# HKUST-Aerial-Robotics/A-LOAM

Measured on AMD Instinct MI355X. Metric: HDL-64 scans/sec (whole node), higher is better.
Workload: dtype f32 features / f64 solve

## Files before the change

a-loam_amd/csrc/capi_internal.hpp:

```cpp
#pragma once
#include <hip/hip_runtime.h>

#include <cstdio>
#include <memory>
#include <string>
#include <utility>
#include <vector>

#include "../../include/aloam_mi355x.h"
#include "aloam_device.hpp"
#include "atlas_kernels.hpp"
#include "checkpoint_kernels.hpp"
#include "export_kernels.hpp"
#include "graphapply_kernels.hpp"
#include "graphmap_kernels.hpp"
#include "graphmarginal_kernels.hpp"
#include "loopreg_kernels.hpp"
#include "loopsearch_kernels.hpp"
#include "mapping_kernels.hpp"
#include "odometry_kernels.hpp"
#include "places_kernels.hpp"
#include "posegraph_kernels.hpp"
#include "registration_kernels.hpp"
#include "relocalize_kernels.hpp"

using namespace aloam;

// ... 350 lines not shown
  if (used[ns]) HIP_TRY(c, hipEventSynchronize(done[ns]));
  *slot = reinterpret_cast<T*>(mem.get() + (size_t)ns * slot_bytes);
  *index = ns;
  return ALOAM_OK;
}
template <int Slots>
int StageRing<Slots>::queue(aloam_ctx* c, int index, const void* src, size_t bytes, void* dst, hipStream_t stream) {
  HIP_TRY(c, hipMemcpyAsync(dst, src, bytes, hipMemcpyHostToDevice, stream));
  HIP_TRY(c, hipEventRecord(done[index], stream));
  used[index] = true;
  return ALOAM_OK;
}

inline float4* cloud_row(const aloam_ctx* c, const ExportSrc& s, int seq) {
  const int r = s.sel == kSelFixed ? 0 : s.sel == kSelCurrent ? c->seq[seq].parity : 1 - c->seq[seq].parity;
  return s.base[r] ? const_cast<float4*>(s.base[r]) + (size_t)seq * s.stride : nullptr;
}

int stage_ints(aloam_ctx* c, const int* src, int n, int* dst);
int check_seq(aloam_ctx* c, int seq);
int require_stage(aloam_ctx* c, int stage);
int check_ids(aloam_ctx* c, const int* ids, int n);
int register_launch(aloam_ctx* c, const void* d_scans, long long seq_stride, const int* n_in, int stride_bytes, int slot = -1, bool debug_arrays = true,
                    const int* n_cols = nullptr);
int stage_batch(aloam_ctx* c, const void* h_scans, long long seq_stride_bytes, size_t row, size_t last, size_t d_seq_stride, int* slot, char** d_in);
int ensure_dense(aloam_ctx* c);
long long cloud_desc(const aloam_ctx* c, int id, ExportSrc* s);
int find_cloud(aloam_ctx* c, int seq, int id, const float4** ptr, int* n);
OdomArgs odom_args(aloam_ctx* c);
MapArgs map_args(aloam_ctx* c);
int grow_map_pool(aloam_ctx* c, long long want, bool clamp);
void queue_map_spill(aloam_ctx* c, const int* mask);
int spill_dropped_since(aloam_ctx* c, long long* fresh);
int atlas_step_check(aloam_ctx* c);
bool queue_atlas_window(aloam_ctx* c, const int* mask);
long long largest_window(const std::vector<int>& keys, const std::vector<int>& counts, const int lo[3], const int hi[3], bool* exact);
KfStore kf_store(aloam_ctx* c);
int keyframe_add_check(aloam_ctx* c, const int* seqs, int n);
void queue_keyframe_capture(aloam_ctx* c, int n);
int queue_keyframe_rewind(aloam_ctx* c, const int* seqs, int n);
int keyframes_dropped_since(aloam_ctx* c, long long* fresh);
inline bool takes_part(const aloam_ctx* c, int b) { return c->all_active || c->seq[b].active; }
struct StageMask {
  std::vector<int> bits;
  const int* dev = nullptr;
  bool any_active = false, any_solve = false, all_solve = true, any_grow = false;
};
int stage_mask(aloam_ctx* c, DevBuf<int>& dst, int (*extra_bits)(const SeqHost&), bool (*unmasked)(const aloam_ctx*, const StageMask&), StageMask* m);
void on_active_mask_set(aloam_ctx* c, const int* active);
void on_frozen_mask_set(aloam_ctx* c, const int* frozen);
int on_slots_reset(aloam_ctx* c, const int* seqs, int n);
void on_slot_loaded(aloam_ctx* c, int seq, bool inited, long long err_events);
void on_sweep_registered(aloam_ctx* c);
void on_odometry_advanced(aloam_ctx* c, const StageMask& m);
void on_last_clouds_replaced(aloam_ctx* c, int seq);
void on_odometry_inputs_replaced(aloam_ctx* c, int seq);
void on_map_corrections_applied(aloam_ctx* c, const int* seqs, int n);
void on_system_inited_forced(aloam_ctx* c, int inited);
int on_map_replaced(aloam_ctx* c, int seq);
int on_map_pool_reallocated(aloam_ctx* c, MapPool&& fresh);
void on_mapping_step_queued(aloam_ctx* c);
int on_atlas_attached(aloam_ctx* c, const std::vector<int>& attached);
void on_places_enabled(aloam_ctx* c);
void on_descriptors_made(aloam_ctx* c, const int* seqs, int n);
void on_graph_nodes_added(aloam_ctx* c, const int* seqs, int n);
void on_graph_edges_added(aloam_ctx* c, int seq, int count);
void on_graph_cleared(aloam_ctx* c, const int* seqs, int n);
int on_graph_applied(aloam_ctx* c, const int* seqs, int n);
long long on_pool_events_reported(aloam_ctx* c, int seq, long long events);
int require_graph(aloam_ctx* c);
const char* graph_edge_check(const aloam_ctx* c, aloam_graph_edge& e, bool measurement);
VoxArgs vox_args(aloam_ctx* c, int n_segs, int levels);
enum CallerMem { kMemPageable, kMemDevice, kMemPinned, kMemManaged, kMemOtherDevice };
CallerMem classify_pointer(const aloam_ctx* c, const void* p, void** dev);
int require_host_list(aloam_ctx* c, const void* p, const char* name);
int export_target(aloam_ctx* c, const void* p, size_t align, const char* what, void** out);
int get_cube_list(aloam_ctx* c, int seq, int which, float* out, int cap_points);
// ... 3 lines not shown
```

a-loam_amd/csrc/capi_odometry.hip:

```cpp
#include <algorithm>
#include <cstring>

#include "capi_internal.hpp"

namespace {

RegArgs reg_args(aloam_ctx* c, const void* d_scans, long long seq_stride, int pt_stride) {
  RegArgs a{};
  a.in = (const char*)d_scans; a.seq_stride = seq_stride; a.pt_stride = pt_stride;
  a.B = c->B; a.cap = c->cap; a.R = c->R; a.NB = c->NB;
  a.ring_from_field = c->cfg.ring_from_field; a.min_range = c->cfg.min_range;
  a.meta = c->d_meta.get(); a.slabs = c->d_slabs.get(); a.slab = c->slab; a.front_lb = c->d_front_lb.get(); a.front_ticket = c->d_front_ticket.get();
  a.ringstart = c->d_ringstart.get(); a.cloud = c->d_cloud.get(); a.curv = c->d_curv.get(); a.label = c->d_label.get();
  a.lookback = c->d_lookback.get(); a.epoch = c->reg_epoch; a.store_debug = c->debug_arrays ? 1 : 0; a.ring_ticket = c->d_ring_ticket.get();
  a.sharp = c->d_sharp.get(); a.flat = c->d_flat.get();
  for (int k = 0; k < 2; ++k) { a.less_sharp[k] = c->d_less_sharp[k].get(); a.less_flat[k] = c->d_less_flat[k].get(); }
  a.active = c->reg_mask;
  return a;
}

}

namespace aloam {

// ... 16 lines not shown
  a.distortion = c->cfg.distortion != 0;
  return a;
}

}

namespace {

int check_batch(aloam_ctx* c, const int* n_in, int stride_bytes) {
  if (const int rc = require_stage(c, ALOAM_STAGE_REGISTRATION)) return rc;
  if (stride_bytes < 12 || (stride_bytes & 3)) { c->err = "stride_bytes must be 12 (x, y, z only) or >= 16, and a multiple of 4"; return ALOAM_E_ARG; }
  if (stride_bytes == 12 && c->cfg.ring_from_field) { c->err = "ring_from_field needs the 4th float of every record: stride_bytes >= 16"; return ALOAM_E_ARG; }
  for (int b = 0; b < c->B; ++b) {
    if (n_in[b] < 0) { c->err = "negative point count"; return ALOAM_E_ARG; }
    if (n_in[b] > c->max_points) { c->err = "scan exceeds max_points"; return ALOAM_E_CAPACITY; }
  }
  return ALOAM_OK;
}

}

namespace aloam {

int register_launch(aloam_ctx* c, const void* d_scans, long long seq_stride, const int* n_in, int stride_bytes, int slot, bool debug_arrays, const int* n_cols) {
  int rc = ALOAM_OK;
  if (!c->all_active && (rc = ensure_dense(c))) return rc;
  c->nin_max = 0;
  for (int b = 0; b < c->B; ++b) if (takes_part(c, b)) c->nin_max = std::max(c->nin_max, n_in[b]);
  if ((rc = stage_ints(c, n_cols ? n_cols : n_in, c->B, c->d_nin.get()))) return rc;
  if (n_cols) c->range_cols.assign(n_cols, n_cols + c->B); else c->range_cols.clear();
  StageMask m;
  rc = stage_mask(c, c->d_mask_reg, [](const SeqHost&) { return 0; }, [](const aloam_ctx* x, const StageMask&) { return x->all_active; }, &m);
  c->reg_mask = m.dev;
  if (rc) return rc;
  on_sweep_registered(c);
  c->debug_arrays = debug_arrays || c->sum_order != 0;
  if (((++c->reg_epoch) & 0x7fffffffu) == 0) ++c->reg_epoch;
  const RegArgs a = reg_args(c, d_scans, seq_stride, stride_bytes);
  if (n_cols) {
    const RangeArgs d{c->d_nin.get(), c->d_rd_az.get(), c->d_rd_rows.get(), c->rd_rows, c->rd_n_az, c->rd_order == ALOAM_RANGE_ROW_MAJOR ? 1 : 0, c->rd_scale};
    { ProfScope p(c, K_FIND_ENDS); launch_find_ends_range(a, d, c->stream); }
    { ProfScope p(c, K_FRONT); launch_front_range(a, d, c->stream); }
  } else {
    { ProfScope p(c, K_FIND_ENDS); launch_find_ends(a, c->d_nin.get(), c->stream); }
    { ProfScope p(c, K_FRONT); launch_front(a, c->stream); }
  }
  { ProfScope p(c, K_RING_STARTS); launch_ring_starts(a, c->stream); }
  c->dense_valid = false;
  if (slot >= 0) { HIP_TRY(c, hipEventRecord(c->in_consumed[slot], c->stream)); c->in_used[slot] = true; }
  { ProfScope p(c, K_RING_FEATURES); launch_ring_features(a, c->npad, 0.2f, c->stream);
    if (c->sum_order) launch_less_flat_reference_order(reg_args(c, d_scans, seq_stride, stride_bytes), c->npad, 0.2f, c->stream); }
  HIP_TRY(c, hipGetLastError());
  c->have_features = true;
  return ALOAM_OK;
}

int ensure_dense(aloam_ctx* c) {
  if (c->dense_valid) return ALOAM_OK;
  { ProfScope p(c, K_DENSE_CLOUD); launch_dense_cloud(reg_args(c, nullptr, 0, 16), c->stream); }
  HIP_TRY(c, hipGetLastError());
  c->dense_valid = true;
  return ALOAM_OK;
}

long long cloud_desc(const aloam_ctx* c, int id, ExportSrc* s) {
  const int* meta = reinterpret_cast<const int*>(c->d_meta.get());
  const int* mseq = reinterpret_cast<const int*>(c->d_mapseq.get());
  const int meta_ints = sizeof(SeqMeta) / sizeof(int), map_ints = sizeof(MapSeq) / sizeof(int);
  const long long sharp = (long long)c->R * kSharpPerRing, flat = (long long)c->R * kFlatPerRing, feat = (long long)c->R * kLessSharpPerRing;
// ... 38 lines not shown
  if (const int rc = c->d_in[s].grow(c, need)) return rc;
  *slot_out = s;
  return ALOAM_OK;
}

int stage_batch(aloam_ctx* c, const void* h_scans, long long seq_stride_bytes, size_t row, size_t last, size_t d_seq_stride, int* slot_out, char** d_in_out) {
  if (seq_stride_bytes < 0) { c->err = "bad stride"; return ALOAM_E_ARG; }
  if (c->B > 1 && (size_t)seq_stride_bytes < row) { c->err = "seq_stride_bytes smaller than a scan"; return ALOAM_E_ARG; }
  int slot = 0;
  if (const int rc = acquire_slab(c, d_seq_stride * c->B, &slot)) return rc;
  char* d_in = c->d_in[slot].get();
  if (row > 0) {
    if (c->B > 1) HIP_TRY(c, hipMemcpy2DAsync(d_in, d_seq_stride, h_scans, (size_t)seq_stride_bytes, row, (size_t)c->B - 1, hipMemcpyHostToDevice, c->copy_stream));
    if (last > 0) HIP_TRY(c, hipMemcpyAsync(d_in + (size_t)(c->B - 1) * d_seq_stride, (const char*)h_scans + (size_t)(c->B - 1) * (size_t)seq_stride_bytes, last, hipMemcpyHostToDevice, c->copy_stream));
  }
  HIP_TRY(c, hipEventRecord(c->in_copied[slot], c->copy_stream));
  HIP_TRY(c, hipStreamWaitEvent(c->stream, c->in_copied[slot], 0));
  *slot_out = slot; *d_in_out = d_in;
  return ALOAM_OK;
}

}

extern "C" {

int aloam_scan_register_device(aloam_ctx* c, const void* d_scans, long long seq_stride_bytes, const int* n_in, int stride_bytes) {
  DeviceScope device_scope(c);
  if (!c || !d_scans || !n_in) return ALOAM_E_ARG;
  if (const int rc = check_batch(c, n_in, stride_bytes)) return rc;
  return register_launch(c, d_scans, seq_stride_bytes, n_in, stride_bytes);
}

int aloam_scan_register(aloam_ctx* c, const void* const* scans, const int* n_in, int stride_bytes) {
  DeviceScope device_scope(c);
  if (!c || !scans || !n_in) return ALOAM_E_ARG;
  int rc = check_batch(c, n_in, stride_bytes);
  if (rc) return rc;
  const size_t seq_stride = (size_t)c->cap * stride_bytes;
  int slot = 0;
  if ((rc = acquire_slab(c, seq_stride * c->B, &slot))) return rc;
  char* d_in = c->d_in[slot].get();
  for (int b = 0; b < c->B; ++b)
    if (n_in[b] > 0) HIP_TRY(c, hipMemcpyAsync(d_in + b * seq_stride, scans[b], (size_t)n_in[b] * stride_bytes, hipMemcpyHostToDevice, c->stream));
  if ((rc = register_launch(c, d_in, (long long)seq_stride, n_in, stride_bytes, slot))) return rc;
  HIP_TRY(c, hipStreamSynchronize(c->stream));
  return ALOAM_OK;
}

static int stage_and_register(aloam_ctx* c, const void* h_scans, long long seq_stride_bytes, const int* n_in, int stride_bytes, bool debug_arrays) {
  if (!c || !h_scans || !n_in) return ALOAM_E_ARG;
  int rc = check_batch(c, n_in, stride_bytes);
  if (rc) return rc;
  const size_t d_seq_stride = (size_t)c->cap * stride_bytes;
  int slot = 0;
  char* d_in = nullptr;
  if ((rc = stage_batch(c, h_scans, seq_stride_bytes, (size_t)*std::max_element(n_in, n_in + c->B) * stride_bytes, (size_t)n_in[c->B - 1] * stride_bytes, d_seq_stride, &slot, &d_in))) return rc;
  return register_launch(c, d_in, (long long)d_seq_stride, n_in, stride_bytes, slot, debug_arrays);
}

int aloam_scan_register_host(aloam_ctx* c, const void* h_scans, long long seq_stride_bytes, const int* n_in, int stride_bytes) {
  DeviceScope device_scope(c);
  return stage_and_register(c, h_scans, seq_stride_bytes, n_in, stride_bytes, true);
}

int aloam_process_host(aloam_ctx* c, const void* h_scans, long long seq_stride_bytes, const int* n_in, int stride_bytes) {
  DeviceScope device_scope(c);
  const int rc = stage_and_register(c, h_scans, seq_stride_bytes, n_in, stride_bytes, false);
  if (rc) return rc;
  return aloam_odometry_step(c);
}

int aloam_input_consumed(aloam_ctx* c) {
  DeviceScope device_scope(c);
  if (!c) return ALOAM_E_ARG;
  for (int s = 0; s < 2; ++s) if (c->in_used[s]) HIP_TRY(c, hipEventSynchronize(c->in_consumed[s]));
  return ALOAM_OK;
}

int aloam_odometry_step(aloam_ctx* c) {
  DeviceScope device_scope(c);
  if (!c) return ALOAM_E_ARG;
  if (const int rc = require_stage(c, ALOAM_STAGE_ODOMETRY)) return rc;
  if (!c->have_features) { c->err = "aloam_odometry_step before any features were registered / set"; return ALOAM_E_STATE; }
  StageMask m;
  if (const int rc = stage_mask(c, c->d_mask_odo, [](const SeqHost& s) { return s.inited ? (int)kSeqSolve : 0; },
                                [](const aloam_ctx* x, const StageMask& k) { return k.all_solve || (!k.any_solve && x->all_active); }, &m)) return rc;
  const int* mask = m.dev;
  const bool any_solve = m.any_solve;
  const bool overlap = c->grid_overlap;
  bool build_last = !overlap;
  if (overlap) for (int b = 0; b < c->B; ++b) build_last |= (m.bits[b] & kSeqSolve) && !c->seq[b].grid_built;
  hipError_t join_err = hipSuccess;
  const int cus = c->gather_blocks / 8;
  auto launch_all = [&]() {
    OdomArgs a = odom_args(c);
    a.active = mask;
    if (overlap) {
      hipError_t e = hipEventRecord(c->grid_fork, c->stream);
      if (e == hipSuccess) e = hipStreamWaitEvent(c->grid_stream, c->grid_fork, 0);
      { ProfScope p(c, K_BUILD_GRIDS, c->grid_stream); launch_build_grids(a, true, cus, c->grid_stream); }
      if (e == hipSuccess) e = hipEventRecord(c->grids_done, c->grid_stream);
      join_err = e;
    }
    if (any_solve && build_last) {
      if (overlap) launch_build_grids(a, false, cus, c->stream);
      else { ProfScope p(c, K_BUILD_GRIDS); launch_build_grids(a, false, cus, c->stream); }
    }
    for (int outer = 0; any_solve && outer < c->cfg.outer_iterations; ++outer) {
      a.outer = outer;
      a.last_outer = outer == c->cfg.outer_iterations - 1;
      { ProfScope p(c, K_TRANSFORM); launch_transform_queries(a, c->stream); }
      { ProfScope p(c, K_ASSOC_CORNER); launch_associate(a, false, c->stream); }
      { ProfScope p(c, K_ASSOC_PLANE); launch_associate(a, true, c->stream); }
      { ProfScope p(c, K_SOLVE); launch_solve(a, c->stream); }
    }
    if (overlap && join_err == hipSuccess) join_err = hipStreamWaitEvent(c->stream, c->grids_done, 0);
    { ProfScope p(c, K_ADVANCE); launch_advance(a, c->stream); }
  };
  if (!any_solve) {
    launch_all();
  } else if (c->use_graph && !c->prof_on && !c->debug_sync) {
    GraphExec& ge = c->odom_graph[mask ? 1 : 0];
    if (!ge) {
      hipGraph_t g = nullptr;
      hipError_t e = hipStreamBeginCapture(c->stream, hipStreamCaptureModeThreadLocal);
      if (e == hipSuccess) {
        launch_all();
        e = hipStreamEndCapture(c->stream, &g);
        if (e == hipSuccess) e = hipGraphInstantiate(&ge.h, g, nullptr, nullptr, 0);
        if (g) (void)hipGraphDestroy(g);
      }
      if (e != hipSuccess) {
        (void)hipGetLastError();
        ge.reset();
        c->use_graph = false;
      }
    }
    if (ge) HIP_TRY(c, hipGraphLaunch(ge, c->stream));
    else launch_all();
  } else {
    launch_all();
  }
  HIP_TRY(c, join_err);
  HIP_TRY(c, hipGetLastError());
  on_odometry_advanced(c, m);
  return ALOAM_OK;
}

int aloam_process_device(aloam_ctx* c, const void* d_scans, long long seq_stride_bytes, const int* n_in, int stride_bytes) {
  DeviceScope device_scope(c);
  if (!c || !d_scans || !n_in) return ALOAM_E_ARG;
  int rc = check_batch(c, n_in, stride_bytes);
  if (rc || (rc = register_launch(c, d_scans, seq_stride_bytes, n_in, stride_bytes, -1, false))) return rc;
  return aloam_odometry_step(c);
}

int aloam_cloud_size(aloam_ctx* c, int seq, int which) {
  DeviceScope device_scope(c);
  const float4* p; int n;
  const int rc = find_cloud(c, seq, which < ALOAM_EXPORT_MAP ? which : -1, &p, &n);
  return rc ? rc : n;
}

int aloam_get_cloud(aloam_ctx* c, int seq, int which, float* out, int cap_points) {
  DeviceScope device_scope(c);
  const float4* p; int n;
  if (const int rc = find_cloud(c, seq, which < ALOAM_EXPORT_MAP ? which : -1, &p, &n)) return rc;
  const int k = n < cap_points ? n : cap_points;
  if (k > 0) HIP_TRY(c, hipMemcpy(out, p, sizeof(float4) * k, hipMemcpyDeviceToHost));
  return n;
}

int aloam_get_pose(aloam_ctx* c, int seq, double q_w[4], double t_w[3], double q_lc[4], double t_lc[3]) {
  DeviceScope device_scope(c);
  int rc = check_seq(c, seq);
  if (rc) return rc;
  OdomState s;
// ... 176 lines not shown
```

a-loam_amd/csrc/capi_seq.hip:

```cpp
#include "capi_internal.hpp"

static int mark_window_stale(aloam_ctx* c, int seq) {
  if (c->any_attached && c->seq[seq].attached) HIP_TRY(c, hipMemsetAsync(c->d_at_stale.get() + seq, 1, sizeof(int), c->stream));
  return ALOAM_OK;
}

namespace aloam {

int stage_mask(aloam_ctx* c, DevBuf<int>& dst, int (*extra_bits)(const SeqHost&), bool (*unmasked)(const aloam_ctx*, const StageMask&), StageMask* m) {
  m->bits.resize(c->B);
  for (int b = 0; b < c->B; ++b) {
    const int v = m->bits[b] = takes_part(c, b) ? (kSeqActive | extra_bits(c->seq[b])) : 0;
    m->any_active |= v != 0; m->any_grow |= (v & kSeqMapGrow) != 0;
    m->any_solve |= (v & kSeqSolve) != 0; m->all_solve &= (v & kSeqSolve) != 0;
  }
  if (unmasked(c, *m)) return ALOAM_OK;
  if (!dst && dmalloc(c, dst, c->B)) return ALOAM_E_HIP;
  if (const int rc = stage_ints(c, m->bits.data(), c->B, dst.get())) return rc;
  m->dev = dst.get();
  return ALOAM_OK;
}

void on_active_mask_set(aloam_ctx* c, const int* active) {
  c->all_active = true;
// ... 22 lines not shown
    SeqHost& s = c->seq[seqs[i]];
    s.parity = 0; s.inited = 0; s.grid_built = false; s.needs_odom = false; s.map_err_seen = 0; s.scorable = false; s.has_sweep = false; s.desc_valid = false;
    s.info_odom = false; s.info_map = false; s.has_stacks = false;
  }
  for (int i = 0; i < n; ++i) if (const int rc = mark_window_stale(c, seqs[i])) return rc;
  return ALOAM_OK;
}

void on_slot_loaded(aloam_ctx* c, int seq, bool inited, long long err_events) {
  SeqHost& s = c->seq[seq];
  s.inited = inited; s.map_err_seen = err_events; s.needs_odom = (c->stages & ALOAM_STAGE_ODOMETRY) != 0;
}

void on_sweep_registered(aloam_ctx* c) {
  const bool odo = c->stages & ALOAM_STAGE_ODOMETRY;
  for (int b = 0; b < c->B; ++b) {
    SeqHost& s = c->seq[b];
    if (odo) s.reg_active = s.active;
    if (takes_part(c, b)) { s.has_sweep = true; s.desc_valid = false; s.info_odom = false; }
  }
  if (odo) c->reg_pending = true;
}

void on_odometry_advanced(aloam_ctx* c, const StageMask& m) {
  for (int b = 0; b < c->B; ++b) {
    SeqHost& s = c->seq[b];
    if (m.bits[b] & kSeqActive) {
      s.parity ^= 1; s.inited = 1; s.needs_odom = false; s.grid_built = c->grid_overlap;
      s.info_odom = (m.bits[b] & kSeqSolve) && c->cfg.outer_iterations > 0;
    }
  }
  c->reg_pending = false;
}

void on_last_clouds_replaced(aloam_ctx* c, int seq) { c->seq[seq].grid_built = false; c->seq[seq].info_odom = false; }
void on_odometry_inputs_replaced(aloam_ctx* c, int seq) { c->seq[seq].info_odom = false; }

int on_map_replaced(aloam_ctx* c, int seq) {
  HIP_TRY(c, hipMemsetAsync(c->d_grid_sig.get() + (size_t)seq * 2, 0, sizeof(MapGridSig) * 2, c->stream));
  c->seq[seq].scorable = false; c->seq[seq].info_map = false;
  return mark_window_stale(c, seq);
}

int on_map_pool_reallocated(aloam_ctx* c, MapPool&& fresh) {
  if (c->d_grid_sig) HIP_TRY(c, hipMemsetAsync(c->d_grid_sig.get(), 0, sizeof(MapGridSig) * c->B * 2, c->stream));
  HIP_TRY(c, hipStreamSynchronize(c->stream));
  c->map = std::move(fresh);
  for (SeqHost& s : c->seq) s.scorable = false;
  return ALOAM_OK;
}

// ... 37 lines not shown
```

a-loam_amd/csrc/odometry_kernels.hip:

```cpp
#include "aloam_device.hpp"
#include "aloam_trig.hpp"
#include "lm_device.hpp"
#include "odometry_solve_device.hpp"
#include "odometry_kernels.hpp"

namespace aloam {

#define ALOAM_PHASE(name) asm volatile("; ##PHASE " name)
#ifdef ALOAM_PHASE_CLOCK
__device__ unsigned long long g_phase_clock_odo[2][32];
#define ALOAM_BG_CLOCK(slot) do { if (threadIdx.x == 0 && blockIdx.x == 1) { atomicAdd(&g_phase_clock_odo[0][slot], (unsigned long long)__builtin_readcyclecounter()); atomicAdd(&g_phase_clock_odo[1][slot], 1ull); } } while (0)
#else
#define ALOAM_BG_CLOCK(slot) do { } while (0)
#endif
#ifdef ALOAM_ASSOC_STATS
__device__ unsigned long long g_assoc_stats[2][32];
#define ALOAM_STAT(cls, i, v) do { if ((threadIdx.x & 63) == 0) atomicAdd(&g_assoc_stats[cls][i], (unsigned long long)(v)); } while (0)
#else
#define ALOAM_STAT(cls, i, v) do { } while (0)
#endif

__device__ __forceinline__ float4 transform_to_start(const float4& p, const OdomState& st) {
  double q[4] = {st.para_q[0], st.para_q[1], st.para_q[2], st.para_q[3]};
  if (q[3] < 0.0) { q[0] = -q[0]; q[1] = -q[1]; q[2] = -q[2]; q[3] = -q[3]; }
// ... 165 lines not shown
#pragma unroll
      for (int t = 0; t < 3; ++t) {
        const unsigned sh = (h[t] & 1u) * 16;
        pos[t] = (atomicAdd(&tab[t * (H / 2) + (h[t] >> 1)], 1u << sh) >> sh) & 0xffffu;
      }
      const float4 e = make_float4(p[u].x, p[u].y, p[u].z, __uint_as_float((unsigned)i | ((unsigned)(key + 1) << 20)));
      g.sorted3[pos[0]] = e;
      g.sorted3c[pos[1]] = e;
      g.sorted2[pos[2]] = e;
    }
  }
  ALOAM_BG_CLOCK(5);
#ifdef ALOAM_PHASE_CLOCK
  __syncthreads();
  ALOAM_BG_CLOCK(6);
#endif
}

__global__ __launch_bounds__(1024) void k_build_grids_fused(OdomArgs a) { build_grids_fused<false>(a, blockIdx.y, blockIdx.x); }
__global__ __launch_bounds__(1024) void k_build_grids_fused_next(OdomArgs a) {
  const int G = gridDim.x;
  for (int r = 0, i = blockIdx.x; i < 2 * a.B; ++r, i += G) {
    build_grids_fused<true>(a, i >> 1, (i ^ r) & 1);
    __syncthreads();
  }
}

constexpr int kBgWaves = 4;
constexpr int kBgUnroll = 4;
template <bool NEXT>
__device__ __forceinline__ void build_grids(const OdomArgs& a) {
  constexpr int U = kBgUnroll;
  const int b = blockIdx.y, which = blockIdx.x / 3, tid = threadIdx.x;
  const int pass_lo = blockIdx.x % 3, pass_hi = pass_lo + 1;
  if (seq_idle(a.active, b, NEXT ? kSeqActive : kSeqSolve)) return;
  const SeqMeta m = a.meta[b];
  const BuildSrc<NEXT> src(a, m, b, which);
  const int n = src.n;
  const float4* pts = src.pts;
  const GridView g = grid_view(a, b, which, src.set);
  if (fused_takes(n, g.H)) return;
  extern __shared__ __attribute__((aligned(16))) int lds[];
  int* cnt = lds;
  int* part = lds + g.H;
  int* s_flag = part + 1024;
  if (tid < 2) s_flag[tid] = n >= (1 << 20) && tid == 0 ? 1 : 0;
// ... 901 lines not shown
  }
}

__global__ void k_advance(SeqMeta* meta, OdomState* state, const int* active, int B) {
  const int b = blockIdx.x * blockDim.x + threadIdx.x;
  if (b >= B || seq_idle(active, b)) return;
  SeqMeta& m = meta[b];
  m.n_corner_last = m.n_less_sharp; m.n_surf_last = m.n_less_flat; m.parity ^= 1;
  state[b].inited = 1;
}
__global__ void k_set_inited(OdomState* state, int B, int inited) {
  const int b = blockIdx.x * blockDim.x + threadIdx.x;
  if (b < B) state[b].inited = inited;
}
void launch_set_inited(OdomState* state, int B, int inited, hipStream_t s) { hipLaunchKernelGGL(k_set_inited, dim3((B + 63) / 64), dim3(64), 0, s, state, B, inited); }
void launch_advance(const OdomArgs& a, hipStream_t s) { hipLaunchKernelGGL(k_advance, dim3((a.B + 63) / 64), dim3(64), 0, s, a.meta, a.state, a.active, a.B); }

size_t build_grids_lds_bytes(int H, int R) { return sizeof(int) * ((size_t)H + 1024 + 2 * (R + 8) + 4); }
static size_t build_grids_fused_lds_bytes(int H) { return sizeof(int) * (3 * (size_t)(H / 2) + 48 + 8 + 2 * kWalkKeys); }
int prepare_build_grids(int H_surf) {
  const int fused = (int)build_grids_fused_lds_bytes(kFusedMaxH), per_grid = (int)build_grids_lds_bytes(H_surf, kMaxRings);
  if (hipFuncSetAttribute((const void*)k_build_grids_fused, hipFuncAttributeMaxDynamicSharedMemorySize, fused) != hipSuccess) return -1;
  if (hipFuncSetAttribute((const void*)k_build_grids_fused_next, hipFuncAttributeMaxDynamicSharedMemorySize, fused) != hipSuccess) return -1;
  if (hipFuncSetAttribute((const void*)k_build_grids, hipFuncAttributeMaxDynamicSharedMemorySize, per_grid) != hipSuccess) return -1;
  return hipFuncSetAttribute((const void*)k_build_grids_next, hipFuncAttributeMaxDynamicSharedMemorySize, per_grid) == hipSuccess ? 0 : -1;
}
void launch_build_grids(const OdomArgs& a, bool next, int cus, hipStream_t s) {
  const int hc = a.grid_H_corner <= kFusedMaxH ? a.grid_H_corner : 0, hs = a.grid_H_surf <= kFusedMaxH ? a.grid_H_surf : 0;
  const size_t fused = build_grids_fused_lds_bytes(hc > hs ? hc : hs), per_grid = build_grids_lds_bytes(a.grid_H_surf, a.R);
  if (next) {
    const int wgs = cus / 2 >= 2 ? (cus / 2) & ~1 : 2;
    if (hc || hs) hipLaunchKernelGGL(k_build_grids_fused_next, dim3(2 * a.B < wgs ? 2 * a.B : wgs), dim3(1024), fused, s, a);
    hipLaunchKernelGGL(k_build_grids_next, dim3(6, a.B), dim3(1024), per_grid, s, a);
  } else {
    if (hc || hs) hipLaunchKernelGGL(k_build_grids_fused, dim3(2, a.B), dim3(1024), fused, s, a);
    hipLaunchKernelGGL(k_build_grids, dim3(6, a.B), dim3(1024), per_grid, s, a);
  }
}
void launch_transform_queries(const OdomArgs& a, hipStream_t s) {
  const dim3 grid((a.R * (kSharpPerRing + kFlatPerRing) + 255) / 256, a.B);
  if (a.distortion) hipLaunchKernelGGL(k_transform_queries<true>, grid, dim3(256), 0, s, a);
  else hipLaunchKernelGGL(k_transform_queries<false>, grid, dim3(256), 0, s, a);
}
void launch_associate(const OdomArgs& a, bool plane, hipStream_t s) {
  const int by = (a.B + 7) / 8 * 8;
  const int qcap = plane ? a.R * kFlatPerRing : a.R * kSharpPerRing;
  const bool wide = a.R > 64;
  const dim3 grid((unsigned)(qcap / 2 * by)), block(64), gridf((unsigned)a.B), blockf(256);
  const dim3 gridn((unsigned)((qcap / 2 + kPairsPerWave - 1) / kPairsPerWave), (unsigned)a.B);
  if (wide) {
    if (plane) { hipLaunchKernelGGL((k_associate_pair<true, true>), grid, block, 0, s, a); hipLaunchKernelGGL((k_associate_nearly<true, true>), gridn, block, 0, s, a); hipLaunchKernelGGL((k_associate_flagged<true, true>), gridf, blockf, 0, s, a); }
    else { hipLaunchKernelGGL((k_associate_pair<false, true>), grid, block, 0, s, a); hipLaunchKernelGGL((k_associate_nearly<false, true>), gridn, block, 0, s, a); hipLaunchKernelGGL((k_associate_flagged<false, true>), gridf, blockf, 0, s, a); }
  } else {
    if (plane) { hipLaunchKernelGGL((k_associate_pair<true, false>), grid, block, 0, s, a); hipLaunchKernelGGL((k_associate_nearly<true, false>), gridn, block, 0, s, a); hipLaunchKernelGGL((k_associate_flagged<true, false>), gridf, blockf, 0, s, a); }
    else { hipLaunchKernelGGL((k_associate_pair<false, false>), grid, block, 0, s, a); hipLaunchKernelGGL((k_associate_nearly<false, false>), gridn, block, 0, s, a); hipLaunchKernelGGL((k_associate_flagged<false, false>), gridf, blockf, 0, s, a); }
  }
}
void launch_solve(const OdomArgs& a, hipStream_t s) {
  if (a.distortion) hipLaunchKernelGGL(k_solve<true>, dim3(a.B), dim3(kSolveThreads), 0, s, a);
// ... 11 lines not shown
```

a-loam_amd/csrc/odometry_kernels.hpp:

```cpp
#pragma once
#include "aloam_device.hpp"

struct aloam_pose_information;

namespace aloam {
size_t build_grids_lds_bytes(int H, int R);
int prepare_build_grids(int H_surf);
void launch_build_grids(const OdomArgs& a, bool next, int cus, hipStream_t s);
void launch_transform_queries(const OdomArgs& a, hipStream_t s);
void launch_associate(const OdomArgs& a, bool plane, hipStream_t s);
void launch_solve(const OdomArgs& a, hipStream_t s);
void launch_advance(const OdomArgs& a, hipStream_t s);
void launch_pose_information_odom(const OdomArgs& a, const int* list, int n, aloam_pose_information* dst, hipStream_t s);
void launch_set_inited(OdomState* state, int B, int inited, hipStream_t s);
}
```

a-loam_amd/csrc/registration_kernels.hip:

```cpp
#include "aloam_device.hpp"
#include "registration_kernels.hpp"
#include "voxel_device.hpp"

namespace aloam {

struct RecordLoader {
  static constexpr bool kKeepPoint = true;
  const char* in; int stride;
  __device__ __forceinline__ float4 operator()(int i) const { return load_point(in, i, stride); }
};

#ifndef ALOAM_RANGE_KEEP_POINT
#define ALOAM_RANGE_KEEP_POINT 0
#endif
struct RangeLoader {
  static constexpr bool kKeepPoint = ALOAM_RANGE_KEEP_POINT;
  const unsigned short* az; const unsigned short* range;
  const float2* az_xy; const float* tab;
  unsigned div, magic; int n_az; bool row_major; float scale;
  __device__ __forceinline__ float4 operator()(int i) const {
#ifdef ALOAM_RANGE_PHASES
    asm volatile("; ##PHASE decode");
#endif
    const unsigned code = range[i];
// ... 30 lines not shown
  __shared__ int s_first, s_last;
  if (tid == 0) { s_first = 0x7fffffff; s_last = -1; }
  __syncthreads();
  for (int base = 0; base < n; base += 4096) {
    bool any = false;
#pragma unroll
    for (int k = 0; k < 4; ++k) {
      const int i = base + k * 1024 + tid;
      if (i < n && point_kept(load(i), a.min_range)) { atomicMin(&s_first, i); any = true; }
    }
    if (__syncthreads_or(any)) break;
  }
  for (int base = 0; base < n; base += 4096) {
    bool any = false;
#pragma unroll
    for (int k = 0; k < 4; ++k) {
      const int i = n - 1 - (base + k * 1024 + tid);
      if (i >= 0 && point_kept(load(i), a.min_range)) { atomicMax(&s_last, i); any = true; }
    }
    if (__syncthreads_or(any)) break;
  }
  __syncthreads();
  if (tid == 0) {
    SeqMeta m = a.meta[b];
    m.n_in = n;
    m.first_kept = s_first;
    m.last_kept = s_last;
    m.half_idx = 0x7fffffff;
    m.err = 0;
    m.n_cloud = 0;
    m.start_ori = 0.f;
    m.end_ori = 0.f;
    if (s_last < 0) {
      m.err = kErrEmpty;
    } else {
      const float4 p0 = load(s_first);
      const float4 p1 = load(s_last);
      const float startOri = -atan2f_port(p0.y, p0.x);
      float endOri = (float)((double)(-atan2f_port(p1.y, p1.x)) + 2 * M_PI);
      if ((double)(endOri - startOri) > 3 * M_PI) endOri = (float)((double)endOri - 2 * M_PI);
      else if ((double)(endOri - startOri) < M_PI) endOri = (float)((double)endOri + 2 * M_PI);
      m.start_ori = startOri;
      m.end_ori = endOri;
    }
    if (n > a.cap) m.err |= kErrPointCap;
    a.meta[b] = m;
  }
}
__global__ __launch_bounds__(1024) void k_find_ends(RegArgs a, const int* __restrict__ n_in) {
  const int b = blockIdx.x;
  if (seq_idle(a.active, b)) return;
  find_ends_body(a, b, n_in[b], RecordLoader{a.in + (long long)b * a.seq_stride, a.pt_stride});
}

__device__ __forceinline__ int ring_from_angle(float angle, int R) {
  int scanID;
  if (R == 16) {
    scanID = (int)((double)((angle + 15) / 2) + 0.5);
    return (scanID > R - 1 || scanID < 0) ? -1 : scanID;
  }
  if (R == 32) {
    scanID = (int)(((double)angle + 92.0 / 3.0) * 3.0 / 4.0);
    return (scanID > R - 1 || scanID < 0) ? -1 : scanID;
  }
  if ((double)angle >= -8.83) scanID = (int)((double)(2 - angle) * 3.0 + 0.5);
  else scanID = R / 2 + (int)((-8.83 - (double)angle) * 2.0 + 0.5);
  if ((double)angle > 2 || (double)angle < -24.33 || scanID > 50 || scanID < 0) return -1;
  return scanID;
}
// ... 769 lines not shown
```

Measured before the change: 133,300.

## Overlap last-cloud grid build with scan registration on a side stream

In the fused process paths, when sequences need their previous-cloud grids built, the build is forked onto the grid stream right after the registration front kernel. It runs with a fixed workgroup budget, so it overlaps the rest of registration instead of running serially at the start of odometry. The odometry step then skips its own next-grid overlap and joins the fork before advancing. This adds a new persistent 'last' kernel variant and a std::function callback, and risks contention between the two streams. It also makes find_ends write only the SeqMeta fields it changes, through a reference, instead of copying the whole struct.

```diff
diff --git a/a-loam_amd/csrc/capi_internal.hpp b/a-loam_amd/csrc/capi_internal.hpp
--- a/a-loam_amd/csrc/capi_internal.hpp
+++ b/a-loam_amd/csrc/capi_internal.hpp
@@ -3,6 +3,7 @@
 
 #include <cstdio>
 #include <memory>
+#include <functional>
 #include <string>
 #include <utility>
 #include <vector>
@@ -399,7 +400,7 @@
 int require_stage(aloam_ctx* c, int stage);
 int check_ids(aloam_ctx* c, const int* ids, int n);
 int register_launch(aloam_ctx* c, const void* d_scans, long long seq_stride, const int* n_in, int stride_bytes, int slot = -1, bool debug_arrays = true,
-                    const int* n_cols = nullptr);
+                    const int* n_cols = nullptr, const std::function<void()>* after_front = nullptr);
 int stage_batch(aloam_ctx* c, const void* h_scans, long long seq_stride_bytes, size_t row, size_t last, size_t d_seq_stride, int* slot, char** d_in);
 int ensure_dense(aloam_ctx* c);
 long long cloud_desc(const aloam_ctx* c, int id, ExportSrc* s);
@@ -429,7 +430,7 @@
 int on_slots_reset(aloam_ctx* c, const int* seqs, int n);
 void on_slot_loaded(aloam_ctx* c, int seq, bool inited, long long err_events);
 void on_sweep_registered(aloam_ctx* c);
-void on_odometry_advanced(aloam_ctx* c, const StageMask& m);
+void on_odometry_advanced(aloam_ctx* c, const StageMask& m, bool built_next);
 void on_last_clouds_replaced(aloam_ctx* c, int seq);
 void on_odometry_inputs_replaced(aloam_ctx* c, int seq);
 void on_map_corrections_applied(aloam_ctx* c, const int* seqs, int n);
diff --git a/a-loam_amd/csrc/capi_odometry.hip b/a-loam_amd/csrc/capi_odometry.hip
--- a/a-loam_amd/csrc/capi_odometry.hip
+++ b/a-loam_amd/csrc/capi_odometry.hip
@@ -1,5 +1,6 @@
 #include <algorithm>
 #include <cstring>
+#include <functional>
 
 #include "capi_internal.hpp"
 
@@ -62,7 +63,8 @@
 
 namespace aloam {
 
-int register_launch(aloam_ctx* c, const void* d_scans, long long seq_stride, const int* n_in, int stride_bytes, int slot, bool debug_arrays, const int* n_cols) {
+int register_launch(aloam_ctx* c, const void* d_scans, long long seq_stride, const int* n_in, int stride_bytes, int slot, bool debug_arrays, const int* n_cols,
+                    const std::function<void()>* after_front) {
   int rc = ALOAM_OK;
   if (!c->all_active && (rc = ensure_dense(c))) return rc;
   c->nin_max = 0;
@@ -85,6 +87,7 @@
     { ProfScope p(c, K_FIND_ENDS); launch_find_ends(a, c->d_nin.get(), c->stream); }
     { ProfScope p(c, K_FRONT); launch_front(a, c->stream); }
   }
+  if (after_front) (*after_front)();
   { ProfScope p(c, K_RING_STARTS); launch_ring_starts(a, c->stream); }
   c->dense_valid = false;
   if (slot >= 0) { HIP_TRY(c, hipEventRecord(c->in_consumed[slot], c->stream)); c->in_used[slot] = true; }
@@ -169,89 +172,92 @@
 
 }
 
-extern "C" {
-
-int aloam_scan_register_device(aloam_ctx* c, const void* d_scans, long long seq_stride_bytes, const int* n_in, int stride_bytes) {
-  DeviceScope device_scope(c);
-  if (!c || !d_scans || !n_in) return ALOAM_E_ARG;
-  if (const int rc = check_batch(c, n_in, stride_bytes)) return rc;
-  return register_launch(c, d_scans, seq_stride_bytes, n_in, stride_bytes);
-}
-
-int aloam_scan_register(aloam_ctx* c, const void* const* scans, const int* n_in, int stride_bytes) {
-  DeviceScope device_scope(c);
-  if (!c || !scans || !n_in) return ALOAM_E_ARG;
-  int rc = check_batch(c, n_in, stride_bytes);
-  if (rc) return rc;
-  const size_t seq_stride = (size_t)c->cap * stride_bytes;
-  int slot = 0;
-  if ((rc = acquire_slab(c, seq_stride * c->B, &slot))) return rc;
-  char* d_in = c->d_in[slot].get();
-  for (int b = 0; b < c->B; ++b)
-    if (n_in[b] > 0) HIP_TRY(c, hipMemcpyAsync(d_in + b * seq_stride, scans[b], (size_t)n_in[b] * stride_bytes, hipMemcpyHostToDevice, c->stream));
-  if ((rc = register_launch(c, d_in, (long long)seq_stride, n_in, stride_bytes, slot))) return rc;
-  HIP_TRY(c, hipStreamSynchronize(c->stream));
-  return ALOAM_OK;
-}
-
-static int stage_and_register(aloam_ctx* c, const void* h_scans, long long seq_stride_bytes, const int* n_in, int stride_bytes, bool debug_arrays) {
-  if (!c || !h_scans || !n_in) return ALOAM_E_ARG;
-  int rc = check_batch(c, n_in, stride_bytes);
-  if (rc) return rc;
-  const size_t d_seq_stride = (size_t)c->cap * stride_bytes;
-  int slot = 0;
-  char* d_in = nullptr;
-  if ((rc = stage_batch(c, h_scans, seq_stride_bytes, (size_t)*std::max_element(n_in, n_in + c->B) * stride_bytes, (size_t)n_in[c->B - 1] * stride_bytes, d_seq_stride, &slot, &d_in))) return rc;
-  return register_launch(c, d_in, (long long)d_seq_stride, n_in, stride_bytes, slot, debug_arrays);
-}
-
-int aloam_scan_register_host(aloam_ctx* c, const void* h_scans, long long seq_stride_bytes, const int* n_in, int stride_bytes) {
-  DeviceScope device_scope(c);
-  return stage_and_register(c, h_scans, seq_stride_bytes, n_in, stride_bytes, true);
-}
-
-int aloam_process_host(aloam_ctx* c, const void* h_scans, long long seq_stride_bytes, const int* n_in, int stride_bytes) {
-  DeviceScope device_scope(c);
-  const int rc = stage_and_register(c, h_scans, seq_stride_bytes, n_in, stride_bytes, false);
-  if (rc) return rc;
-  return aloam_odometry_step(c);
-}
-
-int aloam_input_consumed(aloam_ctx* c) {
-  DeviceScope device_scope(c);
-  if (!c) return ALOAM_E_ARG;
-  for (int s = 0; s < 2; ++s) if (c->in_used[s]) HIP_TRY(c, hipEventSynchronize(c->in_consumed[s]));
-  return ALOAM_OK;
-}
-
-int aloam_odometry_step(aloam_ctx* c) {
-  DeviceScope device_scope(c);
-  if (!c) return ALOAM_E_ARG;
+namespace {
+
+struct GridFork {
+  aloam_ctx* c;
+  bool open = false;
+  hipError_t err = hipSuccess;
+  explicit GridFork(aloam_ctx* c_) : c(c_) {}
+  GridFork(const GridFork&) = delete;
+  GridFork& operator=(const GridFork&) = delete;
+  ~GridFork() { join(); }
+  void note(hipError_t e) { if (err == hipSuccess) err = e; }
+  void begin() {
+    const hipError_t e = hipEventRecord(c->grid_fork, c->stream);
+    note(e);
+    if (e == hipSuccess) note(hipStreamWaitEvent(c->grid_stream, c->grid_fork, 0));
+    open = true;
+  }
+  void launched() { note(hipEventRecord(c->grids_done, c->grid_stream)); }
+  void join() {
+    if (open && err == hipSuccess) note(hipStreamWaitEvent(c->stream, c->grids_done, 0));
+    open = false;
+  }
+};
+
+constexpr int kGridWgsBesideRegistration = 96;
+
+struct OdomStep {
+  StageMask m;
+  bool masked = false;
+  bool beside_registration = false;
+  bool build = false;
+  GridFork fork;
+  explicit OdomStep(aloam_ctx* c) : fork(c) {}
+};
+
+int odometry_mask(aloam_ctx* c, OdomStep* st) {
+  if (const int rc = stage_mask(c, c->d_mask_odo, [](const SeqHost& s) { return s.inited ? (int)kSeqSolve : 0; },
+                                [](const aloam_ctx* x, const StageMask& k) { return k.all_solve || (!k.any_solve && x->all_active); }, &st->m)) return rc;
+  st->masked = true;
+  return ALOAM_OK;
+}
+
+int odometry_begin(aloam_ctx* c, OdomStep* st) {
+  if (!(c->stages & ALOAM_STAGE_ODOMETRY) || !c->grid_overlap) return ALOAM_OK;
+  if (const int rc = odometry_mask(c, st)) return rc;
+  st->beside_registration = true;
+  for (int b = 0; b < c->B; ++b) st->build |= (st->m.bits[b] & kSeqSolve) && !c->seq[b].grid_built;
+  return ALOAM_OK;
+}
+
+void odometry_fork_build(aloam_ctx* c, OdomStep* st) {
+  OdomArgs a = odom_args(c);
+  a.active = st->m.dev;
+  st->fork.begin();
+  { ProfScope p(c, K_BUILD_GRIDS, c->grid_stream); launch_build_grids(a, GridBuild::kPersistentLast, kGridWgsBesideRegistration, c->grid_stream); }
+  st->fork.launched();
+}
+
+int register_with_step(aloam_ctx* c, OdomStep* st, const void* d_scans, long long seq_stride, const int* n_in, int stride_bytes, int slot) {
+  const std::function<void()> fork = [c, st]() { odometry_fork_build(c, st); };
+  return register_launch(c, d_scans, seq_stride, n_in, stride_bytes, slot, false, nullptr, st->build ? &fork : nullptr);
+}
+
+int odometry_finish(aloam_ctx* c, OdomStep* st) {
   if (const int rc = require_stage(c, ALOAM_STAGE_ODOMETRY)) return rc;
   if (!c->have_features) { c->err = "aloam_odometry_step before any features were registered / set"; return ALOAM_E_STATE; }
-  StageMask m;
-  if (const int rc = stage_mask(c, c->d_mask_odo, [](const SeqHost& s) { return s.inited ? (int)kSeqSolve : 0; },
-                                [](const aloam_ctx* x, const StageMask& k) { return k.all_solve || (!k.any_solve && x->all_active); }, &m)) return rc;
+  if (!st->masked) if (const int rc = odometry_mask(c, st)) return rc;
+  const StageMask& m = st->m;
   const int* mask = m.dev;
   const bool any_solve = m.any_solve;
-  const bool overlap = c->grid_overlap;
-  bool build_last = !overlap;
+  st->fork.join();
+  const bool overlap = c->grid_overlap && !st->beside_registration;
+  bool build_last = !c->grid_overlap;
   if (overlap) for (int b = 0; b < c->B; ++b) build_last |= (m.bits[b] & kSeqSolve) && !c->seq[b].grid_built;
-  hipError_t join_err = hipSuccess;
   const int cus = c->gather_blocks / 8;
   auto launch_all = [&]() {
     OdomArgs a = odom_args(c);
     a.active = mask;
     if (overlap) {
-      hipError_t e = hipEventRecord(c->grid_fork, c->stream);
-      if (e == hipSuccess) e = hipStreamWaitEvent(c->grid_stream, c->grid_fork, 0);
-      { ProfScope p(c, K_BUILD_GRIDS, c->grid_stream); launch_build_grids(a, true, cus, c->grid_stream); }
-      if (e == hipSuccess) e = hipEventRecord(c->grids_done, c->grid_stream);
-      join_err = e;
+      st->fork.begin();
+      { ProfScope p(c, K_BUILD_GRIDS, c->grid_stream); launch_build_grids(a, GridBuild::kPersistentNext, cus / 2, c->grid_stream); }
+      st->fork.launched();
     }
     if (any_solve && build_last) {
-      if (overlap) launch_build_grids(a, false, cus, c->stream);
-      else { ProfScope p(c, K_BUILD_GRIDS); launch_build_grids(a, false, cus, c->stream); }
+      if (overlap) launch_build_grids(a, GridBuild::kSerialLast, 0, c->stream);
+      else { ProfScope p(c, K_BUILD_GRIDS); launch_build_grids(a, GridBuild::kSerialLast, 0, c->stream); }
     }
     for (int outer = 0; any_solve && outer < c->cfg.outer_iterations; ++outer) {
       a.outer = outer;
@@ -261,7 +267,7 @@
       { ProfScope p(c, K_ASSOC_PLANE); launch_associate(a, true, c->stream); }
       { ProfScope p(c, K_SOLVE); launch_solve(a, c->stream); }
     }
-    if (overlap && join_err == hipSuccess) join_err = hipStreamWaitEvent(c->stream, c->grids_done, 0);
+    st->fork.join();
     { ProfScope p(c, K_ADVANCE); launch_advance(a, c->stream); }
   };
   if (!any_solve) {
@@ -288,18 +294,86 @@
   } else {
     launch_all();
   }
-  HIP_TRY(c, join_err);
+  HIP_TRY(c, st->fork.err);
   HIP_TRY(c, hipGetLastError());
-  on_odometry_advanced(c, m);
-  return ALOAM_OK;
+  on_odometry_advanced(c, m, overlap);
+  return ALOAM_OK;
+}
+
+}
+
+extern "C" {
+
+int aloam_scan_register_device(aloam_ctx* c, const void* d_scans, long long seq_stride_bytes, const int* n_in, int stride_bytes) {
+  DeviceScope device_scope(c);
+  if (!c || !d_scans || !n_in) return ALOAM_E_ARG;
+  if (const int rc = check_batch(c, n_in, stride_bytes)) return rc;
+  return register_launch(c, d_scans, seq_stride_bytes, n_in, stride_bytes);
+}
+
+int aloam_scan_register(aloam_ctx* c, const void* const* scans, const int* n_in, int stride_bytes) {
+  DeviceScope device_scope(c);
+  if (!c || !scans || !n_in) return ALOAM_E_ARG;
+  int rc = check_batch(c, n_in, stride_bytes);
+  if (rc) return rc;
+  const size_t seq_stride = (size_t)c->cap * stride_bytes;
+  int slot = 0;
+  if ((rc = acquire_slab(c, seq_stride * c->B, &slot))) return rc;
+  char* d_in = c->d_in[slot].get();
+  for (int b = 0; b < c->B; ++b)
+    if (n_in[b] > 0) HIP_TRY(c, hipMemcpyAsync(d_in + b * seq_stride, scans[b], (size_t)n_in[b] * stride_bytes, hipMemcpyHostToDevice, c->stream));
+  if ((rc = register_launch(c, d_in, (long long)seq_stride, n_in, stride_bytes, slot))) return rc;
+  HIP_TRY(c, hipStreamSynchronize(c->stream));
+  return ALOAM_OK;
+}
+
+static int stage_and_register(aloam_ctx* c, const void* h_scans, long long seq_stride_bytes, const int* n_in, int stride_bytes, bool debug_arrays, OdomStep* step = nullptr) {
+  if (!c || !h_scans || !n_in) return ALOAM_E_ARG;
+  int rc = check_batch(c, n_in, stride_bytes);
+  if (rc || (step && (rc = odometry_begin(c, step)))) return rc;
+  const size_t d_seq_stride = (size_t)c->cap * stride_bytes;
+  int slot = 0;
+  char* d_in = nullptr;
+  if ((rc = stage_batch(c, h_scans, seq_stride_bytes, (size_t)*std::max_element(n_in, n_in + c->B) * stride_bytes, (size_t)n_in[c->B - 1] * stride_bytes, d_seq_stride, &slot, &d_in))) return rc;
+  if (step) return register_with_step(c, step, d_in, (long long)d_seq_stride, n_in, stride_bytes, slot);
+  return register_launch(c, d_in, (long long)d_seq_stride, n_in, stride_bytes, slot, debug_arrays);
+}
+
+int aloam_scan_register_host(aloam_ctx* c, const void* h_scans, long long seq_stride_bytes, const int* n_in, int stride_bytes) {
+  DeviceScope device_scope(c);
+  return stage_and_register(c, h_scans, seq_stride_bytes, n_in, stride_bytes, true);
+}
+
+int aloam_process_host(aloam_ctx* c, const void* h_scans, long long seq_stride_bytes, const int* n_in, int stride_bytes) {
+  DeviceScope device_scope(c);
+  if (!c) return ALOAM_E_ARG;
+  OdomStep st(c);
+  if (const int rc = stage_and_register(c, h_scans, seq_stride_bytes, n_in, stride_bytes, false, &st)) return rc;
+  return odometry_finish(c, &st);
+}
+
+int aloam_input_consumed(aloam_ctx* c) {
+  DeviceScope device_scope(c);
+  if (!c) return ALOAM_E_ARG;
+  for (int s = 0; s < 2; ++s) if (c->in_used[s]) HIP_TRY(c, hipEventSynchronize(c->in_consumed[s]));
+  return ALOAM_OK;
+}
+
+int aloam_odometry_step(aloam_ctx* c) {
+  DeviceScope device_scope(c);
+  if (!c) return ALOAM_E_ARG;
+  OdomStep st(c);
+  return odometry_finish(c, &st);
 }
 
 int aloam_process_device(aloam_ctx* c, const void* d_scans, long long seq_stride_bytes, const int* n_in, int stride_bytes) {
   DeviceScope device_scope(c);
   if (!c || !d_scans || !n_in) return ALOAM_E_ARG;
   int rc = check_batch(c, n_in, stride_bytes);
-  if (rc || (rc = register_launch(c, d_scans, seq_stride_bytes, n_in, stride_bytes, -1, false))) return rc;
-  return aloam_odometry_step(c);
+  if (rc) return rc;
+  OdomStep st(c);
+  if ((rc = odometry_begin(c, &st)) || (rc = register_with_step(c, &st, d_scans, seq_stride_bytes, n_in, stride_bytes, -1))) return rc;
+  return odometry_finish(c, &st);
 }
 
 int aloam_cloud_size(aloam_ctx* c, int seq, int which) {
diff --git a/a-loam_amd/csrc/capi_seq.hip b/a-loam_amd/csrc/capi_seq.hip
--- a/a-loam_amd/csrc/capi_seq.hip
+++ b/a-loam_amd/csrc/capi_seq.hip
@@ -68,11 +68,11 @@
   if (odo) c->reg_pending = true;
 }
 
-void on_odometry_advanced(aloam_ctx* c, const StageMask& m) {
+void on_odometry_advanced(aloam_ctx* c, const StageMask& m, bool built_next) {
   for (int b = 0; b < c->B; ++b) {
     SeqHost& s = c->seq[b];
     if (m.bits[b] & kSeqActive) {
-      s.parity ^= 1; s.inited = 1; s.needs_odom = false; s.grid_built = c->grid_overlap;
+      s.parity ^= 1; s.inited = 1; s.needs_odom = false; s.grid_built = built_next;
       s.info_odom = (m.bits[b] & kSeqSolve) && c->cfg.outer_iterations > 0;
     }
   }
diff --git a/a-loam_amd/csrc/odometry_kernels.hip b/a-loam_amd/csrc/odometry_kernels.hip
--- a/a-loam_amd/csrc/odometry_kernels.hip
+++ b/a-loam_amd/csrc/odometry_kernels.hip
@@ -211,6 +211,14 @@
   const int G = gridDim.x;
   for (int r = 0, i = blockIdx.x; i < 2 * a.B; ++r, i += G) {
     build_grids_fused<true>(a, i >> 1, (i ^ r) & 1);
+    __syncthreads();
+  }
+}
+
+__global__ __launch_bounds__(1024) void k_build_grids_fused_last(OdomArgs a) {
+  const int G = gridDim.x;
+  for (int r = 0, i = blockIdx.x; i < 2 * a.B; ++r, i += G) {
+    build_grids_fused<false>(a, i >> 1, (i ^ r) & 1);
     __syncthreads();
   }
 }
@@ -1158,19 +1166,28 @@
   const int fused = (int)build_grids_fused_lds_bytes(kFusedMaxH), per_grid = (int)build_grids_lds_bytes(H_surf, kMaxRings);
   if (hipFuncSetAttribute((const void*)k_build_grids_fused, hipFuncAttributeMaxDynamicSharedMemorySize, fused) != hipSuccess) return -1;
   if (hipFuncSetAttribute((const void*)k_build_grids_fused_next, hipFuncAttributeMaxDynamicSharedMemorySize, fused) != hipSuccess) return -1;
+  if (hipFuncSetAttribute((const void*)k_build_grids_fused_last, hipFuncAttributeMaxDynamicSharedMemorySize, fused) != hipSuccess) return -1;
   if (hipFuncSetAttribute((const void*)k_build_grids, hipFuncAttributeMaxDynamicSharedMemorySize, per_grid) != hipSuccess) return -1;
   return hipFuncSetAttribute((const void*)k_build_grids_next, hipFuncAttributeMaxDynamicSharedMemorySize, per_grid) == hipSuccess ? 0 : -1;
 }
-void launch_build_grids(const OdomArgs& a, bool next, int cus, hipStream_t s) {
+void launch_build_grids(const OdomArgs& a, GridBuild form, int wgs, hipStream_t s) {
   const int hc = a.grid_H_corner <= kFusedMaxH ? a.grid_H_corner : 0, hs = a.grid_H_surf <= kFusedMaxH ? a.grid_H_surf : 0;
   const size_t fused = build_grids_fused_lds_bytes(hc > hs ? hc : hs), per_grid = build_grids_lds_bytes(a.grid_H_surf, a.R);
-  if (next) {
-    const int wgs = cus / 2 >= 2 ? (cus / 2) & ~1 : 2;
-    if (hc || hs) hipLaunchKernelGGL(k_build_grids_fused_next, dim3(2 * a.B < wgs ? 2 * a.B : wgs), dim3(1024), fused, s, a);
-    hipLaunchKernelGGL(k_build_grids_next, dim3(6, a.B), dim3(1024), per_grid, s, a);
-  } else {
-    if (hc || hs) hipLaunchKernelGGL(k_build_grids_fused, dim3(2, a.B), dim3(1024), fused, s, a);
-    hipLaunchKernelGGL(k_build_grids, dim3(6, a.B), dim3(1024), per_grid, s, a);
+  const int even = wgs >= 2 ? wgs & ~1 : 2;
+  const dim3 walk(2 * a.B < even ? 2 * a.B : even);
+  switch (form) {
+    case GridBuild::kPersistentNext:
+      if (hc || hs) hipLaunchKernelGGL(k_build_grids_fused_next, walk, dim3(1024), fused, s, a);
+      hipLaunchKernelGGL(k_build_grids_next, dim3(6, a.B), dim3(1024), per_grid, s, a);
+      break;
+    case GridBuild::kPersistentLast:
+      if (hc || hs) hipLaunchKernelGGL(k_build_grids_fused_last, walk, dim3(1024), fused, s, a);
+      hipLaunchKernelGGL(k_build_grids, dim3(6, a.B), dim3(1024), per_grid, s, a);
+      break;
+    case GridBuild::kSerialLast:
+      if (hc || hs) hipLaunchKernelGGL(k_build_grids_fused, dim3(2, a.B), dim3(1024), fused, s, a);
+      hipLaunchKernelGGL(k_build_grids, dim3(6, a.B), dim3(1024), per_grid, s, a);
+      break;
   }
 }
 void launch_transform_queries(const OdomArgs& a, hipStream_t s) {
diff --git a/a-loam_amd/csrc/odometry_kernels.hpp b/a-loam_amd/csrc/odometry_kernels.hpp
--- a/a-loam_amd/csrc/odometry_kernels.hpp
+++ b/a-loam_amd/csrc/odometry_kernels.hpp
@@ -6,7 +6,8 @@
 namespace aloam {
 size_t build_grids_lds_bytes(int H, int R);
 int prepare_build_grids(int H_surf);
-void launch_build_grids(const OdomArgs& a, bool next, int cus, hipStream_t s);
+enum class GridBuild { kSerialLast, kPersistentNext, kPersistentLast };
+void launch_build_grids(const OdomArgs& a, GridBuild form, int wgs, hipStream_t s);
 void launch_transform_queries(const OdomArgs& a, hipStream_t s);
 void launch_associate(const OdomArgs& a, bool plane, hipStream_t s);
 void launch_solve(const OdomArgs& a, hipStream_t s);
diff --git a/a-loam_amd/csrc/registration_kernels.hip b/a-loam_amd/csrc/registration_kernels.hip
--- a/a-loam_amd/csrc/registration_kernels.hip
+++ b/a-loam_amd/csrc/registration_kernels.hip
@@ -76,17 +76,17 @@
   }
   __syncthreads();
   if (tid == 0) {
-    SeqMeta m = a.meta[b];
+    SeqMeta& m = a.meta[b];
+    int err = 0;
     m.n_in = n;
     m.first_kept = s_first;
     m.last_kept = s_last;
     m.half_idx = 0x7fffffff;
-    m.err = 0;
     m.n_cloud = 0;
     m.start_ori = 0.f;
     m.end_ori = 0.f;
     if (s_last < 0) {
-      m.err = kErrEmpty;
+      err = kErrEmpty;
     } else {
       const float4 p0 = load(s_first);
       const float4 p1 = load(s_last);
@@ -97,8 +97,8 @@
       m.start_ori = startOri;
       m.end_ori = endOri;
     }
-    if (n > a.cap) m.err |= kErrPointCap;
-    a.meta[b] = m;
+    if (n > a.cap) err |= kErrPointCap;
+    m.err = err;
   }
 }
 __global__ __launch_bounds__(1024) void k_find_ends(RegArgs a, const int* __restrict__ n_in) {
```

Measured after the change: 138,400, median of 6. 3.8% higher.
